# okian/kofft

Measured on AMD Instinct MI355X. Metric: batched 4096-pt c32 FFT throughput, GPoints/s (achieved HBM GB/s: roofline.achieved), higher is better.
Workload: dtype f32

## Files before the change

include/kofft_hip.h:

```cpp
#ifndef KOFFT_HIP_H
#define KOFFT_HIP_H

#include <stddef.h>

#ifdef __cplusplus
extern "C" {
#endif

#define KOFFT_OK 0
#define KOFFT_ERR_EMPTY_INPUT 1
#define KOFFT_ERR_NON_POWER_OF_TWO_NO_STD 2
#define KOFFT_ERR_MISMATCHED_LENGTHS 3
#define KOFFT_ERR_INVALID_STRIDE 4
#define KOFFT_ERR_INVALID_HOP_SIZE 5
#define KOFFT_ERR_INVALID_VALUE 6
#define KOFFT_ERR_HIP (-1)
#define KOFFT_ERR_UNSUPPORTED (-2)
#define KOFFT_ERR_NULL (-3)
#define KOFFT_ERR_ALLOC (-4)
#define KOFFT_ERR_RCCL (-5)

typedef struct kofft_hip_ctx kofft_hip_ctx;

const char *kofft_hip_strerror(int status);
// ... 49 lines not shown
int kofft_hip_rfft_f32(kofft_hip_ctx *ctx, const float *in, float *out, const float *window,
                       size_t n, size_t batch);
int kofft_hip_rfft_f32_dev(kofft_hip_ctx *ctx, const float *d_in, float *d_out,
                           const float *d_window, size_t n, size_t batch);
int kofft_hip_irfft_f32(kofft_hip_ctx *ctx, const float *in, float *out, size_t n, size_t batch);
int kofft_hip_irfft_f32_dev(kofft_hip_ctx *ctx, const float *d_in, float *d_out, size_t n,
                            size_t batch);
int kofft_hip_rfft_f64(kofft_hip_ctx *ctx, const double *in, double *out, const double *window,
                       size_t n, size_t batch);
int kofft_hip_rfft_f64_dev(kofft_hip_ctx *ctx, const double *d_in, double *d_out,
                           const double *d_window, size_t n, size_t batch);
int kofft_hip_irfft_f64(kofft_hip_ctx *ctx, const double *in, double *out, size_t n, size_t batch);
int kofft_hip_irfft_f64_dev(kofft_hip_ctx *ctx, const double *d_in, double *d_out, size_t n,
                            size_t batch);

int kofft_hip_dct2_f32(kofft_hip_ctx *ctx, const float *in, float *out, size_t n, size_t batch);
int kofft_hip_dct2_f32_dev(kofft_hip_ctx *ctx, const float *d_in, float *d_out, size_t n, size_t batch);
int kofft_hip_set_dct_fused(kofft_hip_ctx *ctx, int on);

int kofft_hip_hilbert_f32(kofft_hip_ctx *ctx, const float *in, float *out, size_t n, size_t batch);
int kofft_hip_hilbert_f32_dev(kofft_hip_ctx *ctx, const float *d_in, float *d_out, size_t n, size_t batch);
int kofft_hip_set_hilbert_fused(kofft_hip_ctx *ctx, int on);

int kofft_hip_cepstrum_f32(kofft_hip_ctx *ctx, const float *in, float *out, size_t n, size_t batch);
int kofft_hip_cepstrum_f32_dev(kofft_hip_ctx *ctx, const float *d_in, float *d_out, size_t n, size_t batch);
int kofft_hip_set_cepstrum_fused(kofft_hip_ctx *ctx, int on);

int kofft_hip_dct_direct_f32(kofft_hip_ctx *ctx, int type, const float *in, float *out, size_t n, size_t batch);
int kofft_hip_dct_direct_f32_dev(kofft_hip_ctx *ctx, int type, const float *d_in, float *d_out, size_t n, size_t batch);
int kofft_hip_dst_direct_f32(kofft_hip_ctx *ctx, int type, const float *in, float *out, size_t n, size_t batch);
int kofft_hip_dst_direct_f32_dev(kofft_hip_ctx *ctx, int type, const float *d_in, float *d_out, size_t n, size_t batch);
int kofft_hip_set_direct_tiled(kofft_hip_ctx *ctx, int on);
int kofft_hip_set_persist_claim_pct(kofft_hip_ctx *ctx, int pct);
int kofft_hip_dct_direct_table_f32(int type, size_t n, float *C);
int kofft_hip_dst_direct_table_f32(int type, size_t n, float *C);
int kofft_hip_dst_planner_table_f32(int type, size_t n, float *out);
int kofft_hip_dst_planner_table_f64(int type, size_t n, double *out);

int kofft_hip_czt_f32(kofft_hip_ctx *ctx, const float *in, float *out, size_t n, size_t m, float wr, float wi, float ar, float ai,
                      size_t batch);
int kofft_hip_dev_czt_f32(kofft_hip_ctx *ctx, const float *d_in, float *d_out, size_t n, size_t m, float wr, float wi, float ar, float ai,
                          size_t batch);
int kofft_hip_goertzel_f32(kofft_hip_ctx *ctx, const float *in, float *out, size_t n, size_t batch, float sample_rate,
                           const float *target_freqs, size_t nfreq);
int kofft_hip_dev_goertzel_f32(kofft_hip_ctx *ctx, const float *d_in, float *d_out, size_t n, size_t batch, float sample_rate,
                               const float *target_freqs, size_t nfreq);
int kofft_hip_set_czt_route(kofft_hip_ctx *ctx, int mode);
int kofft_hip_czt_table_f32(size_t n, size_t m, float wr, float wi, float ar, float ai, float *C);
int kofft_hip_goertzel_coeff_f32(size_t n, float sample_rate, const float *target_freqs, size_t nfreq, float *coeff);

int kofft_hip_dht_f32(kofft_hip_ctx *ctx, const float *in, float *out, size_t n, size_t batch);
int kofft_hip_dev_dht_f32(kofft_hip_ctx *ctx, const float *d_in, float *d_out, size_t n, size_t batch);
int kofft_hip_set_dht_table_device(kofft_hip_ctx *ctx, int on);
int kofft_hip_dht_table_f32(size_t n, float *H);
int kofft_hip_libm_trigf(const float *x, size_t count, float *cos_out, float *sin_out);

#define KOFFT_WINDOW_HAMMING 0
#define KOFFT_WINDOW_BLACKMAN 1
#define KOFFT_WINDOW_KAISER 2
#define KOFFT_WINDOW_TUKEY 3
#define KOFFT_WINDOW_BARTLETT 4
#define KOFFT_WINDOW_BOHMAN 5
#define KOFFT_WINDOW_NUTTALL 6
int kofft_hip_window_f32(int kind, size_t len, float param, float *out);

#define KOFFT_WAVELET_HAAR 0
// ... 126 lines not shown
```

kofft_amd/_lib.py:

```python
from __future__ import annotations

import ctypes as C
import os
import re
from pathlib import Path

_PKG = Path(__file__).resolve().parent
LIB_PATH = _PKG / "lib" / "libkofft_hip.so"
HEADER_PATH = _PKG.parent / "include" / "kofft_hip.h"


class LibraryMissing(RuntimeError):
    pass


_c_f = C.POINTER(C.c_float)
_c_d = C.POINTER(C.c_double)
_sz = C.c_size_t
_ctx = C.c_void_p

SIGNATURES = {
    "kofft_hip_strerror": (C.c_char_p, [C.c_int]),
    "kofft_hip_last_error": (C.c_char_p, [_ctx]),
    "kofft_hip_version": (C.c_char_p, []),
# ... 24 lines not shown
    "kofft_hip_fft_radix4_c32": (C.c_int, [_ctx, C.c_void_p, _sz, _sz]),
    "kofft_hip_fft_radix4_c64": (C.c_int, [_ctx, C.c_void_p, _sz, _sz]),
    "kofft_hip_fft_radix4_c32_dev": (C.c_int, [_ctx, C.c_void_p, C.c_void_p, _sz, _sz]),
    "kofft_hip_fft_radix4_c64_dev": (C.c_int, [_ctx, C.c_void_p, C.c_void_p, _sz, _sz]),
    "kofft_hip_ifft_radix4_c32": (C.c_int, [_ctx, C.c_void_p, _sz, _sz]),
    "kofft_hip_ifft_radix4_c64": (C.c_int, [_ctx, C.c_void_p, _sz, _sz]),
    "kofft_hip_ifft_radix4_c32_dev": (C.c_int, [_ctx, C.c_void_p, C.c_void_p, _sz, _sz]),
    "kofft_hip_ifft_radix4_c64_dev": (C.c_int, [_ctx, C.c_void_p, C.c_void_p, _sz, _sz]),
    "kofft_hip_fft_c32_strided": (C.c_int, [_ctx, C.c_void_p, _sz, _sz, _sz, C.c_int]),
    "kofft_hip_fft_c64_strided": (C.c_int, [_ctx, C.c_void_p, _sz, _sz, _sz, C.c_int]),
    "kofft_hip_rfft_f32": (C.c_int, [_ctx, C.c_void_p, C.c_void_p, C.c_void_p, _sz, _sz]),
    "kofft_hip_rfft_f32_dev": (C.c_int, [_ctx, C.c_void_p, C.c_void_p, C.c_void_p, _sz, _sz]),
    "kofft_hip_irfft_f32": (C.c_int, [_ctx, C.c_void_p, C.c_void_p, _sz, _sz]),
    "kofft_hip_irfft_f32_dev": (C.c_int, [_ctx, C.c_void_p, C.c_void_p, _sz, _sz]),
    "kofft_hip_rfft_f64": (C.c_int, [_ctx, C.c_void_p, C.c_void_p, C.c_void_p, _sz, _sz]),
    "kofft_hip_rfft_f64_dev": (C.c_int, [_ctx, C.c_void_p, C.c_void_p, C.c_void_p, _sz, _sz]),
    "kofft_hip_irfft_f64": (C.c_int, [_ctx, C.c_void_p, C.c_void_p, _sz, _sz]),
    "kofft_hip_irfft_f64_dev": (C.c_int, [_ctx, C.c_void_p, C.c_void_p, _sz, _sz]),
    "kofft_hip_dct2_f32": (C.c_int, [_ctx, C.c_void_p, C.c_void_p, _sz, _sz]),
    "kofft_hip_dct2_f32_dev": (C.c_int, [_ctx, C.c_void_p, C.c_void_p, _sz, _sz]),
    "kofft_hip_set_dct_fused": (C.c_int, [_ctx, C.c_int]),
    "kofft_hip_hilbert_f32": (C.c_int, [_ctx, C.c_void_p, C.c_void_p, _sz, _sz]),
    "kofft_hip_hilbert_f32_dev": (C.c_int, [_ctx, C.c_void_p, C.c_void_p, _sz, _sz]),
    "kofft_hip_set_hilbert_fused": (C.c_int, [_ctx, C.c_int]),
    "kofft_hip_cepstrum_f32": (C.c_int, [_ctx, C.c_void_p, C.c_void_p, _sz, _sz]),
    "kofft_hip_cepstrum_f32_dev": (C.c_int, [_ctx, C.c_void_p, C.c_void_p, _sz, _sz]),
    "kofft_hip_set_cepstrum_fused": (C.c_int, [_ctx, C.c_int]),
    "kofft_hip_dct_direct_f32": (C.c_int, [_ctx, C.c_int, C.c_void_p, C.c_void_p, _sz, _sz]),
    "kofft_hip_dct_direct_f32_dev": (C.c_int, [_ctx, C.c_int, C.c_void_p, C.c_void_p, _sz, _sz]),
    "kofft_hip_dst_direct_f32": (C.c_int, [_ctx, C.c_int, C.c_void_p, C.c_void_p, _sz, _sz]),
    "kofft_hip_dst_direct_f32_dev": (C.c_int, [_ctx, C.c_int, C.c_void_p, C.c_void_p, _sz, _sz]),
    "kofft_hip_set_direct_tiled": (C.c_int, [_ctx, C.c_int]),
    "kofft_hip_set_persist_claim_pct": (C.c_int, [_ctx, C.c_int]),
    "kofft_hip_dct_direct_table_f32": (C.c_int, [C.c_int, _sz, C.c_void_p]),
    "kofft_hip_dst_direct_table_f32": (C.c_int, [C.c_int, _sz, C.c_void_p]),
    "kofft_hip_dst_planner_table_f32": (C.c_int, [C.c_int, _sz, C.c_void_p]),
    "kofft_hip_dst_planner_table_f64": (C.c_int, [C.c_int, _sz, C.c_void_p]),
    "kofft_hip_czt_f32": (C.c_int, [_ctx, C.c_void_p, C.c_void_p, _sz, _sz, C.c_float, C.c_float, C.c_float, C.c_float, _sz]),
    "kofft_hip_dev_czt_f32": (C.c_int, [_ctx, C.c_void_p, C.c_void_p, _sz, _sz, C.c_float, C.c_float, C.c_float, C.c_float, _sz]),
    "kofft_hip_goertzel_f32": (C.c_int, [_ctx, C.c_void_p, C.c_void_p, _sz, _sz, C.c_float, C.c_void_p, _sz]),
    "kofft_hip_dev_goertzel_f32": (C.c_int, [_ctx, C.c_void_p, C.c_void_p, _sz, _sz, C.c_float, C.c_void_p, _sz]),
    "kofft_hip_set_czt_route": (C.c_int, [_ctx, C.c_int]),
    "kofft_hip_czt_table_f32": (C.c_int, [_sz, _sz, C.c_float, C.c_float, C.c_float, C.c_float, C.c_void_p]),
    "kofft_hip_dht_f32": (C.c_int, [_ctx, C.c_void_p, C.c_void_p, _sz, _sz]),
    "kofft_hip_dev_dht_f32": (C.c_int, [_ctx, C.c_void_p, C.c_void_p, _sz, _sz]),
    "kofft_hip_set_dht_table_device": (C.c_int, [_ctx, C.c_int]),
    "kofft_hip_dht_table_f32": (C.c_int, [_sz, C.c_void_p]),
    "kofft_hip_libm_trigf": (C.c_int, [C.c_void_p, _sz, C.c_void_p, C.c_void_p]),
    "kofft_hip_window_f32": (C.c_int, [C.c_int, _sz, C.c_float, C.c_void_p]),
    "kofft_hip_goertzel_coeff_f32": (C.c_int, [_sz, C.c_float, C.c_void_p, _sz, C.c_void_p]),
    "kofft_hip_dwt_f32": (C.c_int, [_ctx, C.c_int, C.c_void_p, C.c_void_p, C.c_void_p, _sz, _sz]),
    "kofft_hip_dwt_f32_dev": (C.c_int, [_ctx, C.c_int, C.c_void_p, C.c_void_p, C.c_void_p, _sz, _sz]),
    "kofft_hip_idwt_f32": (C.c_int, [_ctx, C.c_int, C.c_void_p, C.c_void_p, C.c_void_p, _sz, _sz]),
    "kofft_hip_idwt_f32_dev": (C.c_int, [_ctx, C.c_int, C.c_void_p, C.c_void_p, C.c_void_p, _sz, _sz]),
    "kofft_hip_dwt_multi_f32": (C.c_int, [_ctx, C.c_int, C.c_void_p, C.c_void_p, C.c_void_p, _sz, _sz, _sz]),
    "kofft_hip_dwt_multi_f32_dev": (C.c_int, [_ctx, C.c_int, C.c_void_p, C.c_void_p, C.c_void_p, _sz, _sz, _sz]),
    "kofft_hip_idwt_multi_f32": (C.c_int, [_ctx, C.c_int, C.c_void_p, C.c_void_p, C.c_void_p, C.c_void_p, _sz, _sz, _sz]),
    "kofft_hip_idwt_multi_f32_dev": (C.c_int, [_ctx, C.c_int, C.c_void_p, C.c_void_p, C.c_void_p, C.c_void_p, _sz, _sz, _sz]),
    "kofft_hip_set_wavelet_fused": (C.c_int, [_ctx, C.c_int]),
    "kofft_hip_dwt_multi_lengths": (C.c_int, [_sz, _sz, C.c_void_p]),
    "kofft_hip_wavelet_taps_f32": (C.c_int, [C.c_int, C.c_int, C.c_void_p, C.c_void_p]),
    "kofft_hip_stft_f32": (C.c_int, [_ctx, C.c_void_p, _sz, C.c_void_p, _sz, _sz, C.c_void_p, _sz]),
    "kofft_hip_stft_parallel_f32": (C.c_int, [_ctx, C.c_void_p, _sz, C.c_void_p, _sz, _sz, C.c_void_p, _sz]),
    "kofft_hip_stft_frame_f32": (C.c_int, [_ctx, C.c_void_p, _sz, C.c_void_p, _sz, _sz, C.c_void_p]),
    "kofft_hip_istft_f32": (C.c_int, [_ctx, C.c_void_p, _sz, C.c_void_p, _sz, _sz, C.c_void_p, _sz, C.c_void_p, _sz]),
    "kofft_hip_istft_parallel_f32": (C.c_int, [_ctx, C.c_void_p, _sz, C.c_void_p, _sz, _sz, C.c_void_p, _sz]),
# ... 78 lines not shown
```

kofft_amd/api.py:

```python
from __future__ import annotations

import ctypes as C
import os
import enum
from typing import Optional, Sequence

import numpy as np

from . import _lib


class FftError(Exception):

    EmptyInput = 1
    NonPowerOfTwoNoStd = 2
    MismatchedLengths = 3
    InvalidStride = 4
    InvalidHopSize = 5
    InvalidValue = 6
    _names = {1: "EmptyInput", 2: "NonPowerOfTwoNoStd", 3: "MismatchedLengths", 4: "InvalidStride",
              5: "InvalidHopSize", 6: "InvalidValue"}

    def __init__(self, code: int):
        self.code = int(code)
# ... 525 lines not shown
            raise ValueError("n and batch are usize in the reference: they cannot be negative")
        self._check(getattr(self._lib, f"kofft_hip_{family}_direct_f32_dev")(self._ctx, int(type), C.c_void_p(d_in), C.c_void_p(d_out),
                                                                             int(n), int(batch)))

    def dct_direct_dev(self, type: int, d_in: int, d_out: int, n: int, batch: int) -> None:
        self._direct_dev("dct", type, d_in, d_out, n, batch)

    def dst_direct_dev(self, type: int, d_in: int, d_out: int, n: int, batch: int) -> None:
        self._direct_dev("dst", type, d_in, d_out, n, batch)

    def set_direct_tiled(self, on: bool) -> None:
        self._check(self._lib.kofft_hip_set_direct_tiled(self._ctx, int(bool(on))))

    def dht_batch(self, x: np.ndarray) -> np.ndarray:
        if self.dtype != np.float32:
            raise TypeError("the Hartley transform is f32-only, like the reference (hartley.rs)")
        a = self._rbuf(x)
        if a.ndim != 2:
            raise TypeError("dht_batch expects a 2-D [batch, n] array")
        out = np.empty(a.shape, np.float32)
        self._check(self._lib.kofft_hip_dht_f32(self._ctx, _ptr(a), _ptr(out), a.shape[1], a.shape[0]))
        return out

    def dht_dev(self, d_in: int, d_out: int, n: int, batch: int) -> None:
        if min(int(n), int(batch)) < 0:
            raise ValueError("n and batch are usize in the reference: they cannot be negative")
        self._check(self._lib.kofft_hip_dev_dht_f32(self._ctx, C.c_void_p(d_in), C.c_void_p(d_out), int(n), int(batch)))

    def set_dht_table_device(self, on: bool) -> None:
        self._check(self._lib.kofft_hip_set_dht_table_device(self._ctx, int(bool(on))))

    def set_persist_claim_pct(self, pct: int) -> None:
        self._check(self._lib.kofft_hip_set_persist_claim_pct(self._ctx, int(pct)))

    def set_czt_route(self, mode: int) -> None:
        self._check(self._lib.kofft_hip_set_czt_route(self._ctx, int(mode)))

    def _spectral_in(self, x, what: str):
        if self.dtype != np.float32:
            raise TypeError(f"{what} is f32-only, like the reference ({what}.rs)")
        dev = hasattr(x, "data_ptr") and hasattr(x, "is_cuda")
        if dev:
            import torch

            if not x.is_cuda or x.dtype != torch.float32:
                raise TypeError(f"{what}: a torch input must be a float32 tensor on the device")
            a = x.contiguous()
        else:
            a = np.ascontiguousarray(x, np.float32)
        if a.ndim not in (1, 2):
            raise TypeError(f"{what} expects a 1-D signal or a 2-D [batch, n] array")
        return (a.reshape(1, -1) if a.ndim == 1 else a), a.ndim == 1, dev

    def czt(self, x, m: int, w, a):
        rows, one, dev = self._spectral_in(x, "czt")
        if int(m) < 0:
            raise ValueError("m is usize in the reference: it cannot be negative")
        m = int(m)
        (wr, wi), (ar, ai) = _complex_pair(w), _complex_pair(a)
        batch, n = rows.shape
        if dev:
            import torch

            out = torch.empty((batch, m, 2), dtype=torch.float32, device=rows.device)
            self._check(self._lib.kofft_hip_dev_czt_f32(self._ctx, C.c_void_p(rows.data_ptr()), C.c_void_p(out.data_ptr()), n, m, wr, wi, ar, ai,
                                                        batch))
# ... 1107 lines not shown
```

kofft_amd/csrc/fft_persist.hip.h:

```cpp
#pragma once

#include "fft_wg.hip.h"

namespace kofft {

template <typename T, int L, int S0, int Q>
__device__ __forceinline__ void load_pass_twiddles(cpx<T> *twr, const int k, const cpx<T> *__restrict__ tw)
{
#pragma unroll
    for (int t = 0; t < Q; ++t) {
#pragma unroll
        for (int h = 0; h < (1 << t); ++h) {
            const int idx = (k << (L - 1 - S0 - t)) + (bitrev(h, t) << (L - 1 - t));
            twr[(1 << t) - 1 + h] = tw[idx];
        }
    }
}

template <typename T, int Q>
__device__ __forceinline__ void reg_pass_r(cpx<T> *v, const cpx<T> *twr)
{
#pragma unroll
    for (int t = 0; t < Q; ++t) {
        const int pos = Q - 1 - t;
#pragma unroll
        for (int h = 0; h < (1 << t); ++h) {
            const cpx<T> w = twr[(1 << t) - 1 + h];
#pragma unroll
            for (int lo = 0; lo < (1 << pos); ++lo) {
                const int c = (h << (pos + 1)) | lo;
                bfly(v[c], v[c | (1 << pos)], w);
            }
        }
    }
// ... 62 lines not shown
    for (int u = 0; u < Gm::R; ++u) p[lds_pad(Gm::out_index(0, u))] = v[u];
}

template <bool WAVE>
__device__ __forceinline__ void exchange_sync()
{
    if constexpr (WAVE) {
        __builtin_amdgcn_fence(__ATOMIC_RELEASE, "wavefront");
        __builtin_amdgcn_wave_barrier();
        __builtin_amdgcn_fence(__ATOMIC_ACQUIRE, "wavefront");
    } else {
        __syncthreads();
    }
}

template <class CFG, class = void>
struct persist_depth { static constexpr int value = 1; };
template <class CFG>
struct persist_depth<CFG, decltype((void)CFG::DEPTH)> { static constexpr int value = CFG::DEPTH; };

template <class CFG, class = void>
struct persist_tw_global { static constexpr bool value = false; };
template <class CFG>
struct persist_tw_global<CFG, decltype((void)CFG::kTwGlobal)> { static constexpr bool value = CFG::kTwGlobal; };

template <class CFG, class = void>
struct persist_claim { static constexpr bool value = false; };
template <class CFG>
struct persist_claim<CFG, decltype((void)CFG::kClaim)> { static constexpr bool value = CFG::kClaim; };

struct PersistClaim {
    unsigned *counters;
    size_t split;
};
template <class IO>
struct PersistClaimIO : IO {
    PersistClaim claim;
};
struct NoXchg {
    __device__ __forceinline__ void put() const {}
    __device__ __forceinline__ void get() const {}
};

#ifdef KOFFT_PERSIST_STAMPS
constexpr int kPersistStampWgs = 4096, kPersistStampWords = 16;
static __device__ unsigned long long g_persist_stamps[kPersistStampWgs * kPersistStampWords];
__device__ __forceinline__ unsigned long long persist_stamp()
{
    unsigned long long t;
    asm volatile("s_memtime %0\n\ts_waitcnt lgkmcnt(0)" : "=s"(t)::"memory");
    return t;
}
__device__ __forceinline__ unsigned long long persist_stamp_real()
{
    unsigned long long t;
    asm volatile("s_memrealtime %0\n\ts_waitcnt lgkmcnt(0)" : "=s"(t)::"memory");
    return t;
}
#endif

template <typename T, int L, int RL, int EPI, class IO, class CFG>
struct PersistState {
    static constexpr int R = 1 << RL;
    static constexpr int NP = (L + RL - 1) / RL;
    static constexpr bool TWG = persist_tw_global<CFG>::value;
    static constexpr bool TW1_REG = !TWG && !(NP == 2 && CFG::kTwLastInLds);
    static constexpr bool TW2_REG = !TWG && NP >= 3 && !(CFG::kTwLastInLds && NP == 3);
// ... 265 lines not shown
        char *extra = smem_raw + (size_t)XPB * NBUF * persist_slot_elems(L) * sizeof(cpx<T>);
        typename IO::Inv *inv_lds = reinterpret_cast<typename IO::Inv *>(extra);
        extra += CFG::kInvInLds ? N * sizeof(typename IO::Inv) : 0;
        cpx<T> *rt_lds = reinterpret_cast<cpx<T> *>(extra);
        extra += (EPI == EPI_RFFT) ? N * sizeof(cpx<T>) : 0;
        cpx<T> *tw_lds = reinterpret_cast<cpx<T> *>(extra);
        if constexpr (CFG::kInvInLds) {
            for (int i = tid; i < N; i += BLOCK) inv_lds[i] = io.invariant(i);
        } else {
#pragma unroll
            for (int u = 0; u < R; ++u) st.inv[u] = io.invariant(FirstG::in_index(0, u) + tau);
        }
        if constexpr (EPI == EPI_RFFT) {
            for (int i = tid; i < N; i += BLOCK) rt_lds[i] = io.rtab[i];
        }
        if constexpr (CFG::kTwLastInLds) {
            for (int i = tid; i < N / 2; i += BLOCK) tw_lds[i] = tw[i];
        }
        st.inv_lds = inv_lds;
        st.rt_lds = rt_lds;
        st.tw_lds = tw_lds;
        if constexpr (CFG::kInvInLds || CFG::kTwLastInLds || EPI == EPI_RFFT) __syncthreads();
    }
    st.g1 = lds_pad(PassGeom<L, RL, 1>::in_index(tau, 0));
    st.g2 = (NP >= 3) ? lds_pad(PassGeom<L, RL, (NP >= 3 ? 2 : 1)>::in_index(tau, 0)) : 0;
    st.g3 = (NP == 4) ? lds_pad(PassGeom<L, RL, NP - 1>::in_index(tau, 0)) : 0;
    st.sc = lds_pad(tau);

    const size_t step = (size_t)gridDim.x * XPB;
    size_t base = (size_t)blockIdx.x * XPB;
    constexpr bool CLAIMS = persist_claim<CFG>::value;
#ifdef KOFFT_PERSIST_STAMPS
    const unsigned long long stamp_entry = persist_stamp(), stamp_entry_real = persist_stamp_real();
    unsigned long long stamp_landed = 0, stamp_landed_real = 0, stamp_rows = 0;
#define KOFFT_PERSIST_STAMP_LANDED()                                                                                  \
    {                                                                                                                 \
        asm volatile("s_waitcnt vmcnt(%0)" ::"n"(RS) : "memory");     \
        stamp_landed = persist_stamp();                                                                               \
        stamp_landed_real = persist_stamp_real();                                                                     \
        __builtin_amdgcn_sched_barrier(0);                                                                            \
    }
#define KOFFT_PERSIST_STAMP_ROW() ++stamp_rows;
#else
#define KOFFT_PERSIST_STAMP_LANDED()
#define KOFFT_PERSIST_STAMP_ROW()
#endif
    [[maybe_unused]] size_t nbase = 0;
    [[maybe_unused]] unsigned long long *claim_word = nullptr;
    if constexpr (CLAIMS) {
        static_assert(NP == 3 && NBUF == 1 && !WAVE && G == 1 && persist_depth<CFG>::value == 1 && !persist_tw_global<CFG>::value &&
                          !(RawSel::pair || RawSel::pair_lds) && !CFG::kInvInLds && !CFG::kTwLastInLds && EPI != EPI_RFFT,
                      "claim hand-out: block-synchronised three-pass transforms, one row ahead, nothing else in LDS");
        claim_word = reinterpret_cast<unsigned long long *>(smem_raw + (size_t)XPB * NBUF * persist_slot_elems(L) * sizeof(cpx<T>));
        const bool first_walked = io.claim.split > 0;
        const bool second_walked = first_walked && base + step < io.claim.split;
        nbase = base + step;
        if (!second_walked) {
            if (tid == 0) {
                size_t r0 = base, r1 = batch;
                if (!first_walked) r0 = io.claim.split + (size_t)XPB * atomicAdd(io.claim.counters, 1u);
                if (r0 < batch) r1 = io.claim.split + (size_t)XPB * atomicAdd(io.claim.counters, 1u);
                claim_word[0] = r0;
                claim_word[1] = r1;
            }
            __syncthreads();
            base = claim_word[0];
            nbase = claim_word[1];
        }
    }
    [[maybe_unused]] auto claim_leave = [&]() {
        if constexpr (CLAIMS) {
            if (tid == 0 && atomicAdd(io.claim.counters + 1, 1u) == gridDim.x - 1) {
                __hip_atomic_store(io.claim.counters, 0u, __ATOMIC_RELAXED, __HIP_MEMORY_SCOPE_AGENT);
                __hip_atomic_store(io.claim.counters + 1, 0u, __ATOMIC_RELAXED, __HIP_MEMORY_SCOPE_AGENT);
            }
        }
    };
    if (base >= batch) {
        if constexpr (CLAIMS) claim_leave();
        return;
    }

    constexpr int DEPTH = persist_depth<CFG>::value;
    static_assert(DEPTH == 1 || DEPTH == 2, "prefetch distance");
    Raw ra[RS], rb[RS];
    const int in_lane_bytes = tau * IO::kRawBytes;
    const int in_row_off = (G == 1) ? 0 : sub * (int)io.in_slot_bytes();
    auto group_cnt = [&](size_t b) -> int {
        const size_t first = b + wslot;
        return first >= batch ? 0 : (batch - first < (size_t)G ? (int)(batch - first) : G);
    };
    auto issue = [&](Raw *dst, const size_t b) {
        const rsrc_t d = io.in_desc_n(b + wslot, group_cnt(b));
        if constexpr (RawSel::pair || RawSel::pair_lds) {
#pragma unroll
            for (int u = 0; u < R; ++u) dst[u] = io.fetch_pair_d(d, in_lane_bytes, FirstG::in_index(0, u), in_row_off);
            dst[R] = io.fetch_last_d(d, in_row_off);
        } else {
#pragma unroll
            for (int u = 0; u < R; ++u) dst[u] = io.fetch_d(d, in_lane_bytes, FirstG::in_index(0, u), in_row_off);
        }
    };
    issue(ra, base);
    typename persist_acc<IO>::type acc{};
    if constexpr (io_has_acc<IO>::value) acc = io.acc_init();
    auto finish = [&]() {
        if constexpr (io_has_acc<IO>::value) io.acc_finish(acc);
        if constexpr (CLAIMS) claim_leave();
#ifdef KOFFT_PERSIST_STAMPS
        if (tid == 0 && blockIdx.x < kPersistStampWgs) {
            unsigned long long *rec = g_persist_stamps + (size_t)blockIdx.x * kPersistStampWords;
            rec[0] = stamp_entry;
            rec[1] = stamp_landed;
            rec[2] = persist_stamp();
            rec[3] = stamp_entry_real;
            rec[4] = stamp_landed_real;
            rec[5] = persist_stamp_real();
            rec[6] = stamp_rows;
            rec[7] = __builtin_amdgcn_s_getreg((31 << 11) | 4);
            rec[8] = __builtin_amdgcn_s_getreg((31 << 11) | 20);
            rec[9] = gridDim.x;
            rec[10] = 1;
        }
#endif
    };

    if constexpr (CLAIMS) {
        unsigned claim_index = 0;
        asm volatile("" : "+v"(claim_index));
        unsigned *const claim_next = io.claim.counters + claim_index;
        struct ClaimXchg {
            unsigned long long *word;
            size_t split;
            const unsigned *ticket;
            size_t *claimed;
            bool writer;
            __device__ __forceinline__ void put() const
            {
                if (writer) *word = split + (size_t)XPB * *ticket;
            }
            __device__ __forceinline__ void get() const { *claimed = *word; }
        };
#define KOFFT_PERSIST_STEP_CLAIM(CUR, NXT, LEAVE)                                                                    \
    {                                                                                                                \
        const bool more = nbase < batch;                                                      \
        const bool walked = nbase + step < io.claim.split;                                    \
        const bool claims = more && !walked && tid == 0;                                                             \
        unsigned ticket;  \
        size_t claimed = batch;                                                                                      \
        if (claims) ticket = atomicAdd(claim_next, 1u);                                                              \
        __builtin_amdgcn_sched_barrier(0);                                   \
        issue(NXT, nbase);                                                                                           \
        __builtin_amdgcn_sched_barrier(0);                           \
        KOFFT_PERSIST_STEP_STAMP                                                                                     \
        const ClaimXchg xchg{claim_word, io.claim.split, &ticket, &claimed, claims};                                 \
        persist_transform<T, L, RL, EPI, CFG>(CUR, st, io, tw, buf0, buf1, base + wslot, group_cnt(base), sub, tau, acc, NoPrefetchParts{}, xchg); \
        KOFFT_PERSIST_STAMP_ROW()                                                                                    \
        if (!more) LEAVE;                                                                                            \
        base = nbase;                                                                                                \
        nbase = walked ? nbase + step : (size_t)claimed;                 \
    }
#define KOFFT_PERSIST_STEP_STAMP KOFFT_PERSIST_STAMP_LANDED()
        KOFFT_PERSIST_STEP_CLAIM(ra, rb, { finish(); return; })
#undef KOFFT_PERSIST_STEP_STAMP
#define KOFFT_PERSIST_STEP_STAMP
        for (;;) {
            KOFFT_PERSIST_STEP_CLAIM(rb, ra, break)
            KOFFT_PERSIST_STEP_CLAIM(ra, rb, break)
        }
#undef KOFFT_PERSIST_STEP_STAMP
        finish();
#undef KOFFT_PERSIST_STEP_CLAIM
    } else if constexpr (DEPTH == 1 && St::TWG && !(RawSel::pair || RawSel::pair_lds)) {
        constexpr bool TOP = persist_twg_top_part(L);
        constexpr int PARTS = TOP ? NP : NP - 1;
#define KOFFT_PERSIST_STEP_PARTS(CUR, NXT, LEAVE)                                                                    \
    {                                                                                                                \
        const size_t nbase = base + step;                                                                            \
        const bool more = nbase < batch;                                                      \
        const rsrc_t nd = io.in_desc_n(nbase + wslot, group_cnt(nbase));                                             \
        auto part = [&](const int i) {                                                                               \
            _Pragma("unroll") for (int u = 0; u < R; ++u)                                                            \
                if (u * PARTS / R == i) NXT[u] = io.fetch_d(nd, in_lane_bytes, FirstG::in_index(0, u), in_row_off);  \
        };                                                                                                           \
        if constexpr (TOP) {                                                                                         \
            part(0);                                                                                                 \
            __builtin_amdgcn_sched_barrier(0);                                                                       \
        }                                                                                                            \
        persist_transform<T, L, RL, EPI, CFG>(CUR, st, io, tw, buf0, buf1, base + wslot, group_cnt(base), sub, tau, acc, part); \
        if (!more) LEAVE;                                                                                            \
        base = nbase;                                                                                                \
    }
        KOFFT_PERSIST_STEP_PARTS(ra, rb, { finish(); return; })
// ... 23 lines not shown
        for (;;) {
            KOFFT_PERSIST_STEP(rb, ra, break)
            KOFFT_PERSIST_STEP(ra, rb, break)
        }
#undef KOFFT_PERSIST_STEP_STAMP
        finish();
#undef KOFFT_PERSIST_STEP
    } else {
        Raw rc[RS];
        issue(rb, base + step);
#define KOFFT_PERSIST_STEP2(CUR, FAR, LEAVE)                                                                         \
    {                                                                                                                \
        const size_t nbase = base + step;                                                                            \
        const bool more = nbase < batch;                                                      \
        issue(FAR, nbase + step);                                                                                    \
        __builtin_amdgcn_sched_barrier(0);                                                                           \
        persist_transform<T, L, RL, EPI, CFG>(CUR, st, io, tw, buf0, buf1, base + wslot, group_cnt(base), sub, tau, acc); \
        if (!more) LEAVE;                                                                                            \
        base = nbase;                                                                                                \
    }
        KOFFT_PERSIST_STEP2(ra, rc, { finish(); return; })
        for (;;) {
            KOFFT_PERSIST_STEP2(rb, ra, break)
            KOFFT_PERSIST_STEP2(rc, rb, break)
            KOFFT_PERSIST_STEP2(ra, rc, break)
        }
        finish();
#undef KOFFT_PERSIST_STEP2
    }
}

#undef KOFFT_PERSIST_STAMP_LANDED
#undef KOFFT_PERSIST_STAMP_ROW

}
```

kofft_amd/csrc/host_common.hip.h:

```cpp
#pragma once

#include "../../include/kofft_hip.h"

#include <hip/hip_runtime.h>

#include <atomic>
#include <cstdio>
#include <cstdlib>
#include <cstring>
#include <map>
#include <new>
#include <string>
#include <utility>
#include <vector>

#include "fft_big.hip.h"
#include "fft_persist.hip.h"
#include "fft_istft.hip.h"
#include "fft_regfile.hip.h"
#include "fft_split_wide.hip.h"
#include "fft_wg.hip.h"
#include "host_layout.h"
#include "tables.h"

#define KOFFT_BIG_PROBE_MAX 8
struct kofft_spectral_slot {
    std::vector<unsigned> key;
    void *d_small = nullptr;
    void *d_table = nullptr;
};
constexpr size_t kSpectralSlots = 4;
struct kofft_hip_ctx {
    int device = 0;
    hipStream_t own_stream = nullptr;
    hipStream_t stream = nullptr;
    hipEvent_t order_event = nullptr;
    int num_cus = 256;
    bool use_persist = true;
    bool istft_fused = true;
    bool dct_fused = true;
    bool hilbert_fused = true;
    bool planar_fused = true;
    bool cepstrum_fused = true;
    bool direct_tiled = true;
    bool dht_table_device = true;
    int wavelet_fused = 1;
    int czt_route = 0;
    bool blue_persist = true;
    int persist_grid_pct = 0;
    int persist_claim_pct = -1;
    unsigned *persist_claim_counters = nullptr;
    bool big_two_only = false;
    int big_three_min = 22;
    bool small32 = true;
    bool big_first11 = true;
    bool big_mid_group = true;
    int big_first_larger = -1;
    bool big_narrow = true;
    int big_narrow_per_cu = 1;
    bool big_persist = true;
    size_t big_persist_min_units = 32;
    int big_first_persist = -1;
    int big_mid_nt = -1;
    bool blue_fused = true;
    bool blue_one_kernel = true;
    bool nd_transpose = true;
    bool nd_fused = true;
    bool nd_two_pass = true;
    int nd_transpose_min = 4096;
    bool zero_copy = true;
    bool host_pipeline = true;
    int host_chunks = 0;
    bool rfft14_wide = true;
    bool rfft13_persist = true;
    int persist64 = 1;
    bool persist_small = true;
    bool rfft_regfile_epi = true;
    bool use_regfile = true;
    bool use_split = true;
    std::string last_error;
    std::map<std::pair<int, size_t>, void *> tables;
    std::vector<kofft_spectral_slot> czt_slots;
    void *goertzel_coeff = nullptr;
// ... 178 lines not shown
        if (arc) return arc;
    }
    const size_t blocks = (batch + XPB - 1) / XPB;
    if (blocks > 0x7fffffffULL) return KOFFT_ERR_UNSUPPORTED;
    hipLaunchKernelGGL(kern, dim3((unsigned)blocks), dim3(BLOCK), lds, ctx->stream, io, tw, batch);
    KOFFT_HIP_TRY(ctx, hipGetLastError());
    return KOFFT_OK;
}

template <int L, class IO> struct PersistCfg;
template <class IO> struct PersistCfgBase {
    static constexpr int NBUF = 1, RL = 4;
    static constexpr bool kInvInLds = IO::kInvInLds, kTwLastInLds = false;
};
template <class IO> struct PersistCfg<13, IO> : PersistCfgBase<IO> { static constexpr int BLOCK = 512, MINW = 2, WG_PER_CU = 1; };
template <bool INV> struct PersistCfg<13, ComplexIO<double, INV>> {
    static constexpr int BLOCK = 512, NBUF = 1, RL = 4, MINW = 2, WG_PER_CU = 1;
    static constexpr bool kInvInLds = false, kTwLastInLds = false, kTwGlobal = true;
};
template <bool INV> struct PersistCfg<12, ComplexIO<double, INV>> {
    static constexpr int BLOCK = 256, NBUF = 1, RL = 4, MINW = 2, WG_PER_CU = 2;
    static constexpr bool kInvInLds = false, kTwLastInLds = false, kTwGlobal = true;
};
#ifndef KOFFT_C12_DEPTH
#define KOFFT_C12_DEPTH 1
#endif
template <class IO> struct PersistCfg<12, IO> : PersistCfgBase<IO> { static constexpr int BLOCK = 256, MINW = 2, WG_PER_CU = 2, DEPTH = KOFFT_C12_DEPTH; };
#ifndef KOFFT_C12_CLAIM
#define KOFFT_C12_CLAIM true
#endif
#ifndef KOFFT_C12_CLAIM_PCT
#define KOFFT_C12_CLAIM_PCT 25
#endif
template <bool INV> struct PersistCfg<12, ComplexIO<float, INV>> : PersistCfgBase<ComplexIO<float, INV>> {
    static constexpr int BLOCK = 256, MINW = 2, WG_PER_CU = 2, DEPTH = KOFFT_C12_DEPTH, kClaimPct = KOFFT_C12_CLAIM_PCT;
    static constexpr bool kClaim = KOFFT_C12_CLAIM;
};
template <class IO> struct PersistCfg<11, IO> : PersistCfgBase<IO> { static constexpr int BLOCK = 256, MINW = 2, WG_PER_CU = 2; };
template <class IO> struct PersistCfg<10, IO> : PersistCfgBase<IO> {
    static constexpr int BLOCK = 256, MINW = IO::kLeanRegisters ? 3 : 2, WG_PER_CU = MINW;
};
#ifndef KOFFT_RFFT10_DEPTH
#define KOFFT_RFFT10_DEPTH 2
#endif
template <> struct PersistCfg<10, RfftIO<float>> : PersistCfgBase<RfftIO<float>> {
    static constexpr int BLOCK = 256, MINW = 2, WG_PER_CU = 2, DEPTH = KOFFT_RFFT10_DEPTH;
};
#ifndef KOFFT_STFT10_DEPTH
#define KOFFT_STFT10_DEPTH 1
#endif
template <> struct PersistCfg<10, StftIO> : PersistCfgBase<StftIO> {
    static constexpr int BLOCK = 256, MINW = 2, WG_PER_CU = 2, DEPTH = KOFFT_STFT10_DEPTH;
};
template <> struct PersistCfg<10, StftMagIO> {
    static constexpr int BLOCK = 256, NBUF = 1, RL = 4, MINW = 3, WG_PER_CU = 3, DEPTH = KOFFT_STFT10_DEPTH;
    static constexpr bool kInvInLds = true, kTwLastInLds = false;
};
#ifndef KOFFT_IRFFT10_WG
#define KOFFT_IRFFT10_WG 2
#endif
#ifndef KOFFT_IRFFT10_DEPTH
#define KOFFT_IRFFT10_DEPTH 1
#endif
#ifndef KOFFT_IRFFT10_TWLDS
#define KOFFT_IRFFT10_TWLDS true
#endif
template <> struct PersistCfg<10, IrfftIO<float>> {
    static constexpr int BLOCK = 256, NBUF = 1, RL = 4, MINW = KOFFT_IRFFT10_WG, WG_PER_CU = KOFFT_IRFFT10_WG, DEPTH = KOFFT_IRFFT10_DEPTH;
// ... 94 lines not shown
    if (blocks > need) blocks = need;
    hipLaunchKernelGGL(kern, dim3((unsigned)blocks), dim3(Cfg::BLOCK), lds, ctx->stream, io, tw, batch);
    KOFFT_HIP_TRY(ctx, hipGetLastError());
    return KOFFT_OK;
    }
}

template <typename T, int L, int EPI, class IO>
int launch_persist_claim(kofft_hip_ctx *ctx, const IO &io, const cpx<T> *tw, size_t batch)
{
    using Cfg = PersistCfg<L, IO>;
    constexpr int RL = Cfg::RL;
    constexpr int XPB = Cfg::BLOCK / ((1 << L) >> RL);
    constexpr size_t lds = (size_t)XPB * Cfg::NBUF * persist_slot_elems(L) * sizeof(cpx<T>) + 16;
    static_assert(lds * Cfg::WG_PER_CU <= 160 * 1024, "LDS budget");
    if (!ctx->persist_claim_counters) {
        ctx->last_error = "the context has no claim counters";
        return KOFFT_ERR_ALLOC;
    }
    using KIO = PersistClaimIO<IO>;
    auto kern = fft_persist_kernel<T, L, RL, EPI, KIO, Cfg>;
    {
        static std::atomic<unsigned long long> attr_done{0};
        const int arc = set_dyn_lds_once(ctx, attr_done, reinterpret_cast<const void *>(kern), lds);
        if (arc) return arc;
    }
    size_t blocks = (size_t)ctx->num_cus * PersistGrid<L, IO>::wg_per_cu(Cfg::WG_PER_CU, batch * sizeof(cpx<T>) << L);
    if (ctx->persist_grid_pct > 0) blocks = blocks * (size_t)ctx->persist_grid_pct / 100;
    if (blocks < 1) blocks = 1;
    const size_t need = (batch + XPB - 1) / XPB;
    if (blocks > need) blocks = need;
    const size_t stride = blocks * XPB;
    const size_t pct = ctx->persist_claim_pct < 0 ? (size_t)Cfg::kClaimPct : (ctx->persist_claim_pct > 100 ? 100 : (size_t)ctx->persist_claim_pct);
    const size_t claimed = batch / 100 * pct + batch % 100 * pct / 100;
    const KIO kio{io, PersistClaim{ctx->persist_claim_counters, (batch - claimed) / stride * stride}};
    hipLaunchKernelGGL(kern, dim3((unsigned)blocks), dim3(Cfg::BLOCK), lds, ctx->stream, kio, tw, batch);
    KOFFT_HIP_TRY(ctx, hipGetLastError());
    return KOFFT_OK;
}

template <typename T, int LA, int LB, class IO>
int launch_split(kofft_hip_ctx *ctx, const IO &io, const cpx<T> *tw, size_t batch)
{
    using Gm = SplitGeom<LA, LB>;
    constexpr size_t lds = 2 * (size_t)Gm::N * sizeof(cpx<T>) + 16;
    static_assert(lds <= 160 * 1024, "LDS budget");
    auto kern = fft_split_persist_kernel<T, LA, LB, IO>;
    {
        static std::atomic<unsigned long long> attr_done{0};
        const int arc = set_dyn_lds_once(ctx, attr_done, reinterpret_cast<const void *>(kern), lds);
        if (arc) return arc;
    }
    size_t blocks = (size_t)ctx->num_cus;
    if (ctx->persist_grid_pct > 0) blocks = blocks * (size_t)ctx->persist_grid_pct / 100;
    if (blocks < 1) blocks = 1;
    if (blocks > batch) blocks = batch;
    hipLaunchKernelGGL(kern, dim3((unsigned)blocks), dim3(Gm::TPT), lds, ctx->stream, io, tw, batch);
    KOFFT_HIP_TRY(ctx, hipGetLastError());
    return KOFFT_OK;
}


template <typename T, int LA, int LB, int QB0, class IO>
int launch_split_wide(kofft_hip_ctx *ctx, const IO &io, const cpx<T> *tw, size_t batch)
{
    using Gm = SplitWideGeom<LA, LB, QB0>;
    constexpr size_t lds = split_wide_lds_bytes<Gm>();
    static_assert(lds <= 160 * 1024, "LDS budget");
// ... 309 lines not shown
```

kofft_amd/csrc/kofft_hip.hip:

```cpp
#include "host_common.hip.h"
#include "host_layout.h"

#include <algorithm>
#include <condition_variable>
#include <mutex>
#include <thread>

using namespace kofft;
using namespace kofft::host;

namespace {

template <class Up, class Run, class Down>
int pipeline_chunks(kofft_hip_ctx *ctx, size_t nchunks, Up up, Run run, Down down)
{
    hipStream_t s_in = nullptr, s_out = nullptr;
    std::vector<hipEvent_t> uploaded(nchunks, nullptr), done(nchunks, nullptr);
    auto cleanup = [&]() {
        for (size_t c = 0; c < nchunks; ++c) {
            if (uploaded[c]) (void)hipEventDestroy(uploaded[c]);
            if (done[c]) (void)hipEventDestroy(done[c]);
        }
        if (s_in) (void)hipStreamDestroy(s_in);
        if (s_out) (void)hipStreamDestroy(s_out);
// ... 839 lines not shown
    return hilbert_host(ctx, in, out, n, batch);
}
int kofft_hip_hilbert_f32_dev(kofft_hip_ctx *ctx, const float *d_in, float *d_out, size_t n, size_t batch)
{
    return hilbert_dev(ctx, d_in, d_out, n, batch);
}
int kofft_hip_set_cepstrum_fused(kofft_hip_ctx *ctx, int on)
{
    if (!ctx) return KOFFT_ERR_NULL;
    ctx->cepstrum_fused = on != 0;
    return KOFFT_OK;
}
int kofft_hip_cepstrum_f32(kofft_hip_ctx *ctx, const float *in, float *out, size_t n, size_t batch)
{
    return cepstrum_host(ctx, in, out, n, batch);
}
int kofft_hip_cepstrum_f32_dev(kofft_hip_ctx *ctx, const float *d_in, float *d_out, size_t n, size_t batch)
{
    return cepstrum_dev(ctx, d_in, d_out, n, batch);
}
int kofft_hip_set_direct_tiled(kofft_hip_ctx *ctx, int on)
{
    if (!ctx) return KOFFT_ERR_NULL;
    ctx->direct_tiled = on != 0;
    return KOFFT_OK;
}
int kofft_hip_set_persist_claim_pct(kofft_hip_ctx *ctx, int pct)
{
    if (!ctx) return KOFFT_ERR_NULL;
    if (pct > 100) return KOFFT_ERR_INVALID_VALUE;
    ctx->persist_claim_pct = pct < 0 ? -1 : pct;
    return KOFFT_OK;
}
int kofft_hip_set_wavelet_fused(kofft_hip_ctx *ctx, int on)
{
    if (!ctx) return KOFFT_ERR_NULL;
    if (on < 0 || on > 2) return KOFFT_ERR_INVALID_VALUE;
    ctx->wavelet_fused = on;
    return KOFFT_OK;
}
int kofft_hip_dwt_f32(kofft_hip_ctx *ctx, int wavelet, const float *in, float *approx, float *detail, size_t len, size_t batch)
{
    return dwt_host(ctx, wavelet, in, approx, detail, len, batch);
}
int kofft_hip_dwt_f32_dev(kofft_hip_ctx *ctx, int wavelet, const float *d_in, float *d_approx, float *d_detail, size_t len, size_t batch)
{
    return dwt_dev(ctx, wavelet, d_in, d_approx, d_detail, len, batch);
}
int kofft_hip_idwt_f32(kofft_hip_ctx *ctx, int wavelet, const float *approx, const float *detail, float *out, size_t n, size_t batch)
{
    return idwt_host(ctx, wavelet, approx, detail, out, n, batch);
}
int kofft_hip_idwt_f32_dev(kofft_hip_ctx *ctx, int wavelet, const float *d_approx, const float *d_detail, float *d_out, size_t n, size_t batch)
{
    return idwt_dev(ctx, wavelet, d_approx, d_detail, d_out, n, batch);
}
int kofft_hip_dwt_multi_f32(kofft_hip_ctx *ctx, int wavelet, const float *in, float *approx, float *details, size_t len, size_t batch,
                            size_t levels)
{
    return dwt_multi_host(ctx, wavelet, in, approx, details, len, batch, levels);
}
int kofft_hip_dwt_multi_f32_dev(kofft_hip_ctx *ctx, int wavelet, const float *d_in, float *d_approx, float *d_details, size_t len,
                                size_t batch, size_t levels)
{
    return dwt_multi_dev(ctx, wavelet, d_in, d_approx, d_details, len, batch, levels);
}
// ... 328 lines not shown
```

Before: 374.2.

## Hand out runs of consecutive rows per claim ticket in persistent FFT

Adds a banded claim schedule in which each atomic ticket can grant a run of several strided rows, encoded in the high bits of the claim word. Rows within a run proceed without another atomicAdd, reducing contention on the claim counter. Claim words are broadcast with readfirstlane. The default run length is 1, which reproduces the previous per-row hand-out, and a setter and compile-time macro allow tuning.

```diff
diff --git a/include/kofft_hip.h b/include/kofft_hip.h
--- a/include/kofft_hip.h
+++ b/include/kofft_hip.h
@@ -105,6 +105,7 @@
 int kofft_hip_dst_direct_f32_dev(kofft_hip_ctx *ctx, int type, const float *d_in, float *d_out, size_t n, size_t batch);
 int kofft_hip_set_direct_tiled(kofft_hip_ctx *ctx, int on);
 int kofft_hip_set_persist_claim_pct(kofft_hip_ctx *ctx, int pct);
+int kofft_hip_set_persist_claim_run(kofft_hip_ctx *ctx, int k0);
 int kofft_hip_dct_direct_table_f32(int type, size_t n, float *C);
 int kofft_hip_dst_direct_table_f32(int type, size_t n, float *C);
 int kofft_hip_dst_planner_table_f32(int type, size_t n, float *out);
diff --git a/kofft_amd/_lib.py b/kofft_amd/_lib.py
--- a/kofft_amd/_lib.py
+++ b/kofft_amd/_lib.py
@@ -80,6 +80,7 @@
     "kofft_hip_dst_direct_f32_dev": (C.c_int, [_ctx, C.c_int, C.c_void_p, C.c_void_p, _sz, _sz]),
     "kofft_hip_set_direct_tiled": (C.c_int, [_ctx, C.c_int]),
     "kofft_hip_set_persist_claim_pct": (C.c_int, [_ctx, C.c_int]),
+    "kofft_hip_set_persist_claim_run": (C.c_int, [_ctx, C.c_int]),
     "kofft_hip_dct_direct_table_f32": (C.c_int, [C.c_int, _sz, C.c_void_p]),
     "kofft_hip_dst_direct_table_f32": (C.c_int, [C.c_int, _sz, C.c_void_p]),
     "kofft_hip_dst_planner_table_f32": (C.c_int, [C.c_int, _sz, C.c_void_p]),
diff --git a/kofft_amd/api.py b/kofft_amd/api.py
--- a/kofft_amd/api.py
+++ b/kofft_amd/api.py
@@ -581,6 +581,9 @@
 
     def set_persist_claim_pct(self, pct: int) -> None:
         self._check(self._lib.kofft_hip_set_persist_claim_pct(self._ctx, int(pct)))
+
+    def set_persist_claim_run(self, k0: int) -> None:
+        self._check(self._lib.kofft_hip_set_persist_claim_run(self._ctx, int(k0)))
 
     def set_czt_route(self, mode: int) -> None:
         self._check(self._lib.kofft_hip_set_czt_route(self._ctx, int(mode)))
diff --git a/kofft_amd/csrc/claim_runs.h b/kofft_amd/csrc/claim_runs.h
--- /dev/null
+++ b/kofft_amd/csrc/claim_runs.h
@@ -0,0 +1,83 @@
+#pragma once
+#include <cstddef>
+
+#if defined(__HIPCC__) || defined(__CUDACC__)
+#define KOFFT_CLAIM_HD __host__ __device__
+#else
+#define KOFFT_CLAIM_HD
+#endif
+
+namespace kofft {
+namespace claim {
+
+constexpr unsigned kMaxRun = 64;
+
+KOFFT_CLAIM_HD constexpr bool valid_run(long k0) { return k0 >= 0 && k0 <= (long)kMaxRun && (k0 & (k0 - 1)) == 0; }
+
+KOFFT_CLAIM_HD constexpr unsigned log2_run(unsigned k0)
+{
+    unsigned l = 0;
+    while ((2u << l) <= k0) ++l;
+    return l;
+}
+
+struct Schedule {
+    unsigned grid;
+    unsigned lg;
+};
+
+KOFFT_CLAIM_HD constexpr unsigned band_rounds(unsigned lg, unsigned b) { return b < lg ? (1u << lg) >> b : 1u; }
+KOFFT_CLAIM_HD constexpr size_t band_first_round(unsigned lg, size_t b)
+{
+    const size_t k2 = size_t(2) << lg;
+    return b <= lg ? k2 - (k2 >> b) : k2 - 1 + (b - lg - 1);
+}
+
+struct Span {
+    size_t first;
+    unsigned rounds;
+};
+KOFFT_CLAIM_HD inline Span ticket_span(const Schedule s, size_t split, unsigned xpb, unsigned t)
+{
+    const unsigned band = t / s.grid, col = t - band * s.grid;
+    const size_t stride = (size_t)s.grid * xpb;
+    return Span{split + (size_t)col * xpb + stride * band_first_round(s.lg, band), band_rounds(s.lg, band)};
+}
+
+struct Run {
+    size_t first;
+    unsigned rows;
+};
+KOFFT_CLAIM_HD inline Run ticket_run(const Schedule s, size_t split, size_t batch, unsigned xpb, unsigned t)
+{
+    const Span sp = ticket_span(s, split, xpb, t);
+    if (sp.first >= batch) return Run{sp.first, 0u};
+    const size_t stride = (size_t)s.grid * xpb;
+    const size_t fit = (batch - sp.first + stride - 1) / stride;
+    return Run{sp.first, fit < sp.rounds ? (unsigned)fit : sp.rounds};
+}
+
+KOFFT_CLAIM_HD inline size_t split_of(size_t batch, size_t stride, size_t pct)
+{
+    const size_t claimed = batch / 100 * pct + batch % 100 * pct / 100;
+    return (batch - claimed) / stride * stride;
+}
+
+KOFFT_CLAIM_HD inline size_t region_rounds(size_t split, size_t batch, size_t stride) { return batch > split ? (batch - split + stride - 1) / stride : 0; }
+
+KOFFT_CLAIM_HD inline size_t used_bands(unsigned lg, size_t rounds)
+{
+    size_t b = 0;
+    while (band_first_round(lg, b) < rounds) ++b;
+    return b;
+}
+
+KOFFT_CLAIM_HD inline unsigned default_run(unsigned want, size_t rounds)
+{
+    unsigned k0 = 1;
+    while (k0 * 2 <= want && k0 * 2 <= kMaxRun && (size_t)k0 * 4 - 1 <= rounds) k0 *= 2;
+    return k0;
+}
+
+}
+}
diff --git a/kofft_amd/csrc/fft_persist.hip.h b/kofft_amd/csrc/fft_persist.hip.h
--- a/kofft_amd/csrc/fft_persist.hip.h
+++ b/kofft_amd/csrc/fft_persist.hip.h
@@ -1,5 +1,6 @@
 #pragma once
 
+#include "claim_runs.h"
 #include "fft_wg.hip.h"
 
 namespace kofft {
@@ -128,7 +129,20 @@
 struct PersistClaim {
     unsigned *counters;
     size_t split;
+    unsigned run_lg;
 };
+constexpr int kClaimRowBits = 56;
+__device__ __forceinline__ unsigned long long persist_claim_pack(const claim::Schedule sched, const size_t split, const size_t batch, const unsigned xpb,
+                                                                 const unsigned ticket)
+{
+    const claim::Span sp = claim::ticket_span(sched, split, xpb, ticket);
+    return sp.first >= batch ? (unsigned long long)batch : (unsigned long long)sp.first | (unsigned long long)(sp.rounds - 1) << kClaimRowBits;
+}
+__device__ __forceinline__ unsigned long long persist_uniform64(const unsigned long long v)
+{
+    const unsigned lo = __builtin_amdgcn_readfirstlane((unsigned)v), hi = __builtin_amdgcn_readfirstlane((unsigned)(v >> 32));
+    return (unsigned long long)hi << 32 | lo;
+}
 template <class IO>
 struct PersistClaimIO : IO {
     PersistClaim claim;
@@ -460,7 +474,7 @@
     constexpr bool CLAIMS = persist_claim<CFG>::value;
 #ifdef KOFFT_PERSIST_STAMPS
     const unsigned long long stamp_entry = persist_stamp(), stamp_entry_real = persist_stamp_real();
-    unsigned long long stamp_landed = 0, stamp_landed_real = 0, stamp_rows = 0;
+    unsigned long long stamp_landed = 0, stamp_landed_real = 0, stamp_rows = 0, stamp_claims = 0;
 #define KOFFT_PERSIST_STAMP_LANDED()                                                                                  \
     {                                                                                                                 \
         asm volatile("s_waitcnt vmcnt(%0)" ::"n"(RS) : "memory");     \
@@ -469,31 +483,42 @@
         __builtin_amdgcn_sched_barrier(0);                                                                            \
     }
 #define KOFFT_PERSIST_STAMP_ROW() ++stamp_rows;
+#define KOFFT_PERSIST_STAMP_CLAIMS(n) stamp_claims += (n);
 #else
 #define KOFFT_PERSIST_STAMP_LANDED()
 #define KOFFT_PERSIST_STAMP_ROW()
+#define KOFFT_PERSIST_STAMP_CLAIMS(n)
 #endif
     [[maybe_unused]] size_t nbase = 0;
+    [[maybe_unused]] unsigned run_left = 0;
     [[maybe_unused]] unsigned long long *claim_word = nullptr;
+    [[maybe_unused]] claim::Schedule sched{};
     if constexpr (CLAIMS) {
         static_assert(NP == 3 && NBUF == 1 && !WAVE && G == 1 && persist_depth<CFG>::value == 1 && !persist_tw_global<CFG>::value &&
                           !(RawSel::pair || RawSel::pair_lds) && !CFG::kInvInLds && !CFG::kTwLastInLds && EPI != EPI_RFFT,
                       "claim hand-out: block-synchronised three-pass transforms, one row ahead, nothing else in LDS");
         claim_word = reinterpret_cast<unsigned long long *>(smem_raw + (size_t)XPB * NBUF * persist_slot_elems(L) * sizeof(cpx<T>));
+        sched = claim::Schedule{gridDim.x, io.claim.run_lg};
         const bool first_walked = io.claim.split > 0;
         const bool second_walked = first_walked && base + step < io.claim.split;
         nbase = base + step;
         if (!second_walked) {
             if (tid == 0) {
-                size_t r0 = base, r1 = batch;
-                if (!first_walked) r0 = io.claim.split + (size_t)XPB * atomicAdd(io.claim.counters, 1u);
-                if (r0 < batch) r1 = io.claim.split + (size_t)XPB * atomicAdd(io.claim.counters, 1u);
-                claim_word[0] = r0;
+                unsigned long long r0 = base, r1 = batch;
+                if (!first_walked) r0 = persist_claim_pack(sched, io.claim.split, batch, XPB, atomicAdd(io.claim.counters, 1u));
+                const size_t row0 = r0 & ((1ull << kClaimRowBits) - 1);
+                const unsigned after0 = (unsigned)(r0 >> kClaimRowBits);
+                if (after0 != 0 && row0 + step < batch) r1 = (row0 + step) | (unsigned long long)(after0 - 1) << kClaimRowBits;
+                else if (row0 < batch) r1 = persist_claim_pack(sched, io.claim.split, batch, XPB, atomicAdd(io.claim.counters, 1u));
+                KOFFT_PERSIST_STAMP_CLAIMS((first_walked ? 0 : 1) + ((after0 != 0 && row0 + step < batch) || row0 >= batch ? 0 : 1))
+                claim_word[0] = row0;
                 claim_word[1] = r1;
             }
             __syncthreads();
-            base = claim_word[0];
-            nbase = claim_word[1];
+            base = persist_uniform64(claim_word[0]);
+            const unsigned long long second = persist_uniform64(claim_word[1]);
+            nbase = second & ((1ull << kClaimRowBits) - 1);
+            run_left = (unsigned)(second >> kClaimRowBits);
         }
     }
     [[maybe_unused]] auto claim_leave = [&]() {
@@ -549,6 +574,7 @@
             rec[8] = __builtin_amdgcn_s_getreg((31 << 11) | 20);
             rec[9] = gridDim.x;
             rec[10] = 1;
+            rec[11] = stamp_claims;
         }
 #endif
     };
@@ -559,34 +585,48 @@
         unsigned *const claim_next = io.claim.counters + claim_index;
         struct ClaimXchg {
             unsigned long long *word;
-            size_t split;
+            claim::Schedule sched;
+            size_t split, batch;
             const unsigned *ticket;
-            size_t *claimed;
+            unsigned long long *claimed;
+            bool claiming;
             bool writer;
             __device__ __forceinline__ void put() const
             {
-                if (writer) *word = split + (size_t)XPB * *ticket;
-            }
-            __device__ __forceinline__ void get() const { *claimed = *word; }
+                if (writer) *word = persist_claim_pack(sched, split, batch, XPB, *ticket);
+            }
+            __device__ __forceinline__ void get() const
+            {
+                if (claiming) *claimed = persist_uniform64(*word);
+            }
         };
 #define KOFFT_PERSIST_STEP_CLAIM(CUR, NXT, LEAVE)                                                                    \
     {                                                                                                                \
         const bool more = nbase < batch;                                                      \
-        const bool walked = nbase + step < io.claim.split;                                    \
-        const bool claims = more && !walked && tid == 0;                                                             \
+         \
+        const bool cont = nbase + step < io.claim.split || (run_left != 0 && nbase + step < batch);                  \
+        const bool claiming = more && !cont;                                                                         \
+        const bool claims = claiming && tid == 0;                                                                    \
         unsigned ticket;  \
-        size_t claimed = batch;                                                                                      \
+        unsigned long long claimed = batch;                                                                          \
         if (claims) ticket = atomicAdd(claim_next, 1u);                                                              \
+        KOFFT_PERSIST_STAMP_CLAIMS(claiming ? 1 : 0)                                                                 \
         __builtin_amdgcn_sched_barrier(0);                                   \
         issue(NXT, nbase);                                                                                           \
         __builtin_amdgcn_sched_barrier(0);                           \
         KOFFT_PERSIST_STEP_STAMP                                                                                     \
-        const ClaimXchg xchg{claim_word, io.claim.split, &ticket, &claimed, claims};                                 \
+        const ClaimXchg xchg{claim_word, sched, io.claim.split, batch, &ticket, &claimed, claiming, claims};         \
         persist_transform<T, L, RL, EPI, CFG>(CUR, st, io, tw, buf0, buf1, base + wslot, group_cnt(base), sub, tau, acc, NoPrefetchParts{}, xchg); \
         KOFFT_PERSIST_STAMP_ROW()                                                                                    \
         if (!more) LEAVE;                                                                                            \
         base = nbase;                                                                                                \
-        nbase = walked ? nbase + step : (size_t)claimed;                 \
+        if (cont) {                                                                                                  \
+            nbase += step;                                                                                           \
+            run_left -= run_left != 0 ? 1u : 0u;                                                                     \
+        } else {                                      \
+            nbase = (size_t)(claimed & ((1ull << kClaimRowBits) - 1));                                               \
+            run_left = (unsigned)(claimed >> kClaimRowBits);                                                         \
+        }                                                                                                            \
     }
 #define KOFFT_PERSIST_STEP_STAMP KOFFT_PERSIST_STAMP_LANDED()
         KOFFT_PERSIST_STEP_CLAIM(ra, rb, { finish(); return; })
@@ -676,5 +716,6 @@
 
 #undef KOFFT_PERSIST_STAMP_LANDED
 #undef KOFFT_PERSIST_STAMP_ROW
-
-}
+#undef KOFFT_PERSIST_STAMP_CLAIMS
+
+}
diff --git a/kofft_amd/csrc/host_common.hip.h b/kofft_amd/csrc/host_common.hip.h
--- a/kofft_amd/csrc/host_common.hip.h
+++ b/kofft_amd/csrc/host_common.hip.h
@@ -49,6 +49,7 @@
     bool blue_persist = true;
     int persist_grid_pct = 0;
     int persist_claim_pct = -1;
+    int persist_claim_run = -1;
     unsigned *persist_claim_counters = nullptr;
     bool big_two_only = false;
     int big_three_min = 22;
@@ -293,8 +294,12 @@
 #ifndef KOFFT_C12_CLAIM_PCT
 #define KOFFT_C12_CLAIM_PCT 25
 #endif
+#ifndef KOFFT_C12_CLAIM_RUN
+#define KOFFT_C12_CLAIM_RUN 1
+#endif
 template <bool INV> struct PersistCfg<12, ComplexIO<float, INV>> : PersistCfgBase<ComplexIO<float, INV>> {
-    static constexpr int BLOCK = 256, MINW = 2, WG_PER_CU = 2, DEPTH = KOFFT_C12_DEPTH, kClaimPct = KOFFT_C12_CLAIM_PCT;
+    static constexpr int BLOCK = 256, MINW = 2, WG_PER_CU = 2, DEPTH = KOFFT_C12_DEPTH, kClaimPct = KOFFT_C12_CLAIM_PCT, kClaimRun = KOFFT_C12_CLAIM_RUN;
+    static_assert(claim::valid_run(kClaimRun), "KOFFT_C12_CLAIM_RUN: 0, 1 or a power of two up to 64");
     static constexpr bool kClaim = KOFFT_C12_CLAIM;
 };
 template <class IO> struct PersistCfg<11, IO> : PersistCfgBase<IO> { static constexpr int BLOCK = 256, MINW = 2, WG_PER_CU = 2; };
@@ -455,8 +460,10 @@
     if (blocks > need) blocks = need;
     const size_t stride = blocks * XPB;
     const size_t pct = ctx->persist_claim_pct < 0 ? (size_t)Cfg::kClaimPct : (ctx->persist_claim_pct > 100 ? 100 : (size_t)ctx->persist_claim_pct);
-    const size_t claimed = batch / 100 * pct + batch % 100 * pct / 100;
-    const KIO kio{io, PersistClaim{ctx->persist_claim_counters, (batch - claimed) / stride * stride}};
+    const size_t split = claim::split_of(batch, stride, pct);
+    const unsigned k0 = ctx->persist_claim_run >= 0 ? (unsigned)ctx->persist_claim_run
+                                                    : claim::default_run((unsigned)Cfg::kClaimRun, claim::region_rounds(split, batch, stride));
+    const KIO kio{io, PersistClaim{ctx->persist_claim_counters, split, claim::log2_run(k0)}};
     hipLaunchKernelGGL(kern, dim3((unsigned)blocks), dim3(Cfg::BLOCK), lds, ctx->stream, kio, tw, batch);
     KOFFT_HIP_TRY(ctx, hipGetLastError());
     return KOFFT_OK;
diff --git a/kofft_amd/csrc/kofft_hip.hip b/kofft_amd/csrc/kofft_hip.hip
--- a/kofft_amd/csrc/kofft_hip.hip
+++ b/kofft_amd/csrc/kofft_hip.hip
@@ -895,6 +895,13 @@
     ctx->persist_claim_pct = pct < 0 ? -1 : pct;
     return KOFFT_OK;
 }
+int kofft_hip_set_persist_claim_run(kofft_hip_ctx *ctx, int k0)
+{
+    if (!ctx) return KOFFT_ERR_NULL;
+    if (k0 != -1 && !claim::valid_run(k0)) return KOFFT_ERR_INVALID_VALUE;
+    ctx->persist_claim_run = k0;
+    return KOFFT_OK;
+}
 int kofft_hip_set_wavelet_fused(kofft_hip_ctx *ctx, int on)
 {
     if (!ctx) return KOFFT_ERR_NULL;
```

Result: no change. 373.3 (-0.3%).
